# cindytsai/multigrid_poisson_solver

Measured on AMD Instinct MI355X. Metric: vcycle_mlups, higher is better.
Workload: dtype f64; 1 GPU; V(3,3)-cycle N=8192^2 fp64, 11 levels to N=8, red-black GS(1e-7) coarse solve, cycle-file driver (eager, stream smoother: temporally blocked wave-streaming kernels on the large levels, register-tile kernels on the levels 65..1024, one-workgroup LDS kernel below; halos recomputed, neighbours via DPP lane shifts); N=8192, levels=11

## Files before the change

### multigrid_poisson_solver_amd/csrc/mg_stream_impl.h

```cpp
#include <hip/hip_runtime.h>

#include <type_traits>
#include <utility>

#include <algorithm>
#include <cstdlib>
#include <vector>

#include "mg_divconst.h"
#include "mg_internal.h"
#include "mg_lane_ops.h"

#if !defined(MG_REAL) || !defined(MG_REAL_NS)
#error "define MG_REAL (double|float) and MG_REAL_NS (f64|f32) before including mg_stream_impl.h"
#endif

namespace mg {
namespace k {
namespace MG_REAL_NS {

typedef MG_REAL real_t;

constexpr int PF_DEFAULT = 2;
#ifndef MG_WAVES_PER_WG
#define MG_WAVES_PER_WG 4
#endif
constexpr int WAVES_PER_WG = MG_WAVES_PER_WG;
constexpr int MAX_S = 4;
#ifndef MG_PF
#define MG_PF 2
#endif

constexpr bool recompute_instantiated(int pre, int steps)
{
    return MG_PF == 2 && pre >= 1 && steps >= 1 && pre <= MAX_S && steps <= MAX_S && pre + steps <= 6;
}

enum InMode { IN_LOAD = 0, IN_ZERO = 1, IN_PROLONG = 2 };

typedef real_t real2_t __attribute__((ext_vector_type(2)));
typedef real_t real4_t __attribute__((ext_vector_type(4)));

struct StreamParams {
    int N;
    real_t dx2, inv;
    const real_t *in;
    const real_t *F;
    real_t *out;
    real_t *D;
    int d_sign;
    double *part;
    long long *trace;
    int cols4;
    int rows_per_chunk;
    int groups;
    int n_blocks;
    int row_base, rows_local, own_y0, own_y1;
    int norm_y0, norm_y1;
    double *out_wide;
    int coarse_base, coarse_rows;
    int raw_norm;
    int nt_min_n;
    int no_out;
    int pre;
    int fc_base, fc_rows;
    const real_t *coarse;
    int Nc;
    const int *p_orow, *p_ocol;
    const real_t *p_rhi, *p_rlo, *p_chi, *p_clo;
    real_t c_dx, c_dx_rcp;
    real_t *Fc;
    int M;
    const int *r_inv;
    const real_t *r_w;
    const real_t *r_wf;
    const NodeBatchItem *batch;
    int part_stride;
    int n_batch;
    double *const *err_outs;
    real_t cw;
    int wt;
};


typedef const int __attribute__((address_space(4))) *const_int_ptr;
typedef const real_t __attribute__((address_space(4))) *const_real_ptr;
__device__ __forceinline__ int table_i(const int *t, int i) { return ((const_int_ptr)(uintptr_t)t)[i]; }
__device__ __forceinline__ real_t table_d(const real_t *t, int i) { return ((const_real_ptr)(uintptr_t)t)[i]; }

template <int COLS>
struct Row {
    real_t v[COLS];
};

#ifndef MG_ZERO_LEVEL1
#define MG_ZERO_LEVEL1 1
#endif
#ifndef MG_NT_LOADS
#define MG_NT_LOADS 0
#endif
template <int COLS, bool NT = false>
__device__ __forceinline__ Row<COLS> load_row(const real_t *__restrict__ row, unsigned col_bytes)
{
    Row<COLS> r;
    const char *a = reinterpret_cast<const char *>(row) + col_bytes;
    if constexpr (COLS == 2) {
        const real2_t t = NT ? __builtin_nontemporal_load(reinterpret_cast<const real2_t *>(a)) : *reinterpret_cast<const real2_t *>(a);
        r.v[0] = t.x;
        r.v[1] = t.y;
    } else if constexpr (COLS == 4) {
        const real4_t t = NT ? __builtin_nontemporal_load(reinterpret_cast<const real4_t *>(a)) : *reinterpret_cast<const real4_t *>(a);
        r.v[0] = t.x;
        r.v[1] = t.y;
        r.v[2] = t.z;
        r.v[3] = t.w;
    } else {
        r.v[0] = *reinterpret_cast<const real_t *>(a);
    }
    return r;
}

template <int COLS, bool NT>
__device__ __forceinline__ void store_row(real_t *__restrict__ row, unsigned col_bytes, const Row<COLS> &r)
{
    char *a = reinterpret_cast<char *>(row) + col_bytes;
    if constexpr (COLS == 2) {
        real2_t t;
        t.x = r.v[0];
        t.y = r.v[1];
        if constexpr (NT) __builtin_nontemporal_store(t, reinterpret_cast<real2_t *>(a));
        else *reinterpret_cast<real2_t *>(a) = t;
    } else if constexpr (COLS == 4) {
        real4_t t;
        t.x = r.v[0];
        t.y = r.v[1];
        t.z = r.v[2];
        t.w = r.v[3];
        if constexpr (NT) __builtin_nontemporal_store(t, reinterpret_cast<real4_t *>(a));
        else *reinterpret_cast<real4_t *>(a) = t;
    } else {
        *reinterpret_cast<real_t *>(a) = r.v[0];
    }
}

template <int S, bool RESTRICT, int COLS = 2>
struct Halo {
    static constexpr int A = COLS > 2 ? COLS : 2;
    static constexpr int value = (S + (RESTRICT ? 2 : 1) + A - 1) / A * A;
};


template <int NCV>
struct CoarseV {
    real_t v[NCV];
};
template <int NCV>
__device__ __forceinline__ CoarseV<NCV> load_coarse(const real_t *__restrict__ coarse, int Nc, int base, int rows, int row,
                                                    const unsigned (&col)[NCV])
{
    CoarseV<NCV> c;
    int r = row - base;
    r = r < 0 ? 0 : (r < rows - 1 ? r : rows - 1);
    const char *b = reinterpret_cast<const char *>(coarse + (size_t)r * Nc);
#pragma unroll
    for (int q = 0; q < NCV; ++q) c.v[q] = *reinterpret_cast<const real_t *>(b + col[q]);
    return c;
}


template <int NCV>
__device__ __forceinline__ CoarseV<NCV> load_coarse_local(const real_t *__restrict__ coarse, int Nc, int local_row, const unsigned (&col)[NCV])
{
    CoarseV<NCV> c;
    const char *b = reinterpret_cast<const char *>(coarse + (size_t)local_row * Nc);
#pragma unroll
    for (int q = 0; q < NCV; ++q) c.v[q] = *reinterpret_cast<const real_t *>(b + col[q]);
    return c;
}

template <class F, int... K>
__device__ __forceinline__ void unrolled_while(F &&f, std::integer_sequence<int, K...>)
{
    (void)(f(std::integral_constant<int, K>{}) && ...);
}

#ifndef MG_WPE_DOWN
#define MG_WPE_DOWN 0
#endif
template <int S, int COLS, int IN, bool RESTRICT, int PRE>
struct WavesPerSimd {
    static constexpr int min = (MG_WPE_DOWN > 0 && sizeof(real_t) == 8 && COLS == 2 && IN == 1  && RESTRICT && S <= 3) ? MG_WPE_DOWN : 1;
};

#ifndef MG_LDS_RING
#define MG_LDS_RING 1
#endif
#ifndef MG_PACKED_F32
#define MG_PACKED_F32 1
#endif
typedef float pk_t __attribute__((ext_vector_type(2)));
__device__ __forceinline__ pk_t pk(float a, float b)
{
    pk_t r;
    r.x = a;
    r.y = b;
    return r;
}
__device__ __forceinline__ pk_t pk_fma(pk_t a, pk_t b, pk_t c) { return __builtin_elementwise_fma(a, b, c); }
__device__ __forceinline__ pk_t pk_div_by_const(pk_t x, float c, float rc)
{
    const pk_t cc = pk(c, c), rr = pk(rc, rc);
    pk_t q = x * rr;
    pk_t r = pk_fma(-q, cc, x);
    q = pk_fma(r, rr, q);
    r = pk_fma(-q, cc, x);
    return pk_fma(r, rr, q);
}
template <int COLS, int PRE>
struct LdsRing {
    static constexpr bool value = MG_LDS_RING && PRE > 0 && (COLS == 2 || (COLS == 4 && sizeof(real_t) == 4));
};
template <int COLS> struct RingVec { typedef real_t full; typedef real_t half; };
template <> struct RingVec<2> { typedef real2_t full; typedef real_t half; };
template <> struct RingVec<4> { typedef real4_t full; typedef real2_t half; };
template <int COLS>
__device__ __forceinline__ typename RingVec<COLS>::full ring_pack(const Row<COLS> &r)
{
    typename RingVec<COLS>::full t;
    if constexpr (COLS == 1) t = r.v[0];
    else {
#pragma unroll
        for (int j = 0; j < COLS; ++j) t[j] = r.v[j];
    }
    return t;
}
template <int COLS>
__device__ __forceinline__ Row<COLS> ring_unpack(const typename RingVec<COLS>::full &t)
{
    Row<COLS> r;
    if constexpr (COLS == 1) r.v[0] = t;
    else {
#pragma unroll
        for (int j = 0; j < COLS; ++j) r.v[j] = t[j];
    }
    return r;
}
#ifndef MG_PF_UP
#define MG_PF_UP 3
#endif
#ifndef MG_PF_DOWN
#define MG_PF_DOWN 3
#endif
#ifndef MG_WPE_UP
#define MG_WPE_UP 2
#endif

template <int S, int COLS, int IN, bool RESTRICT, int PF = PF_DEFAULT, bool NT = false, int PRE = 0, bool WT = false>
__global__ __launch_bounds__(64 * WAVES_PER_WG) __attribute__((amdgpu_waves_per_eu(LdsRing<COLS, PRE>::value ? MG_WPE_UP : WavesPerSimd<S, COLS, IN, RESTRICT, PRE>::min)))
void k_jacobi_stream(const StreamParams p)
{
    static_assert(COLS == 2 || COLS == 4 || (IN != IN_PROLONG && !RESTRICT), "fused transfer stages need column pairs");
    static_assert(COLS != 4 || sizeof(real_t) == 4, "4 columns per lane = one 16-byte access: fp32 fields only");
    constexpr int NCV = COLS / 2 + 2;
    constexpr int NS = COLS >= 2 ? COLS / 2 : 1;
    static_assert(PRE == 0 || (IN == IN_PROLONG && !RESTRICT), "recomputed pre-smoothing belongs to the fused `1` node");
    static_assert(!WT || (PRE == 0 && sizeof(real_t) == 8), "the weighted sweep: fp64 nodes that store and re-read U");
    constexpr int L = S + PRE;
    constexpr bool LDSR = LdsRing<COLS, PRE>::value;
    constexpr bool HALF = LDSR;
    constexpr bool PACKED = MG_PACKED_F32 && (COLS == 2 || COLS == 4) && sizeof(real_t) == 4;
#ifndef MG_TB_DIRECT
#define MG_TB_DIRECT 0
#endif
    constexpr bool TB_DIRECT = LDSR && MG_TB_DIRECT;
    constexpr int NB = LDSR ? 8 : (PF + L + 2 <= 8 ? 8 : 16);
    constexpr int NFR = LDSR ? (PF < 4 ? 4 : 8) : NB;
    static_assert((LDSR ? L + 2 <= NB : PF + L + 2 <= NB) && PF < 8, "the F ring has NB slots, the U ring 4 or 8");
    static_assert(!LDSR || (IN == IN_PROLONG && !RESTRICT), "the LDS ring belongs to the recomputing `1` node");
    typedef typename RingVec<COLS>::full ring_t;
    typedef typename RingVec<COLS>::half ringh_t;
    __shared__ ring_t s_g[LDSR ? WAVES_PER_WG : 1][LDSR ? NB : 1][LDSR ? 64 : 1];
    __shared__ ringh_t s_f[LDSR ? WAVES_PER_WG : 1][LDSR ? NB : 1][LDSR ? 64 : 1];
    constexpr int W = 64 * COLS;
    constexpr int H = Halo<L, RESTRICT, COLS>::value;
    constexpr int OW = W - 2 * H;

#ifdef MG_STREAM_TRACE
    const long long tr0 = wall_clock64();
#endif
    const int per_xcd = (p.n_blocks + 7) >> 3;
    const int tile = (int)(blockIdx.x & 7) * per_xcd + (int)(blockIdx.x >> 3);
    if (tile >= p.n_blocks) return;
    const real_t *a_in = p.in, *a_F = p.F, *a_coarse = p.coarse;
    real_t *a_out = p.out, *a_Fc = p.Fc;
    double *a_part = p.part;
    if (p.batch) {
        typedef const NodeBatchItem __attribute__((address_space(4))) *item_ptr;
        const item_ptr b = (item_ptr)(uintptr_t)(p.batch + blockIdx.y);
        a_in = static_cast<const real_t *>(b->in);
        a_F = static_cast<const real_t *>(b->F);
        a_coarse = static_cast<const real_t *>(b->coarse);
        a_out = static_cast<real_t *>(b->out);
        a_Fc = static_cast<real_t *>(b->Fc);
        if (a_part) a_part += (size_t)blockIdx.y * (size_t)p.part_stride;
    }
    const int chunk = tile / p.groups;
    const int group = tile - chunk * p.groups;

    const int lane = threadIdx.x & 63;
    const int wave = threadIdx.x >> 6;
    const int strip = group * WAVES_PER_WG + wave;
    const int N = p.N;
    const int own_x0 = strip * OW;
    if (own_x0 >= N) {
        if (a_part && lane == 0) a_part[(size_t)tile * WAVES_PER_WG + wave] = 0.0;
        return;
    }
    const int y0 = p.own_y0 + chunk * p.rows_per_chunk;
    int y1 = y0 + p.rows_per_chunk;
    if (y1 > p.own_y1) y1 = p.own_y1;
    if (y0 >= p.own_y1) return;
    const int av_lo = p.row_base > 0 ? p.row_base : 0;
    const int av_hi = p.row_base + p.rows_local < N ? p.row_base + p.rows_local : N;

    const int xl = own_x0 - H + lane * COLS;
    bool col_in[COLS], col_edge[COLS];
    bool lane_owns = true;
    real_t qc[COLS];
#pragma unroll
    for (int j = 0; j < COLS; ++j) {
        const int x = xl + j;
        col_in[j] = x >= 0 && x < N;
        col_edge[j] = x <= 0 || x >= N - 1;
        lane_owns = lane_owns && x >= own_x0 && x < own_x0 + OW && x < N;
        qc[j] = col_edge[j] ? real_t(0.0) : (WT ? p.cw : real_t(0.25));
    }
    int nm_even[COLS], nm_odd[COLS];
#pragma unroll
    for (int j = 0; j < COLS; ++j) {
        const bool mine = lane_owns && !col_edge[j];
        nm_even[j] = (mine && ((xl + j) & 1) == 0) ? -1 : 0;
        nm_odd[j] = (mine && ((xl + j) & 1) != 0) ? -1 : 0;
    }
    const bool lane_loads = col_in[0] && col_in[COLS - 1];
    const real_t dx2 = p.dx2, inv = p.inv;
    const bool want_res = RESTRICT || p.D != nullptr || p.part != nullptr;
    const unsigned col_off = (unsigned)(xl < 0 ? 0 : (xl > N - COLS ? N - COLS : xl)) * (unsigned)sizeof(real_t);
    const unsigned col_st = (unsigned)(xl < 0 ? 0 : xl) * (unsigned)sizeof(real_t);
    const unsigned row_bytes = (unsigned)N * (unsigned)sizeof(real_t);

    unsigned pc_col[NCV];
    int pc_cell[COLS];
    real_t pc_hi[COLS], pc_lo[COLS];
    real_t hA[COLS], hB[COLS];
#pragma unroll
    for (int q = 0; q < NCV; ++q) pc_col[q] = 0u;
#pragma unroll
    for (int j = 0; j < COLS; ++j) {
        pc_cell[j] = 0;
        pc_hi[j] = pc_lo[j] = hA[j] = hB[j] = real_t(0.0);
    }
    int c_row = -0x40000000;
    if constexpr (IN == IN_PROLONG) {
        if (lane_loads) {
            const int pc_base = p.p_ocol[xl];
            const int last = p.Nc - 1;
#pragma unroll
            for (int j = 0; j < COLS; ++j) {
                pc_cell[j] = p.p_ocol[xl + j] - pc_base;
                pc_hi[j] = p.p_chi[xl + j];
                pc_lo[j] = p.p_clo[xl + j];
            }
#pragma unroll
            for (int q = 0; q < NCV; ++q) pc_col[q] = (unsigned)(pc_base + q < last ? pc_base + q : last) * (unsigned)sizeof(real_t);
        }
    }
    auto interpolate = [&](const CoarseV<NCV> &c, real_t (&h)[COLS]) {
#pragma unroll
        for (int j = 0; j < COLS; ++j) {
            real_t ca = c.v[0], cb = c.v[1];
#pragma unroll
            for (int q = 1; q + 1 < NCV; ++q) {
                const bool here = pc_cell[j] == q;
                ca = here ? c.v[q] : ca;
                cb = here ? c.v[q + 1] : cb;
            }
            h[j] = ca * pc_hi[j] + cb * pc_lo[j];
        }
    };

    int rc_col[NS];
    bool rc_shift[NS];
    real_t rw_a[NS], rw_b[NS];
    Row<COLS> d_prev;
#pragma unroll
    for (int j = 0; j < COLS; ++j) d_prev.v[j] = 0.0;
#pragma unroll
    for (int q = 0; q < NS; ++q) {
        rc_col[q] = -1;
        rc_shift[q] = false;
        rw_a[q] = rw_b[q] = real_t(0.0);
    }
    if constexpr (RESTRICT) {
        if (lane_owns) {
#pragma unroll
            for (int q = 0; q < NS; ++q) {
                const int ca = p.r_inv[xl + 2 * q], cb = p.r_inv[xl + 2 * q + 1];
                rc_col[q] = ca >= 0 ? ca : cb;
                rc_shift[q] = ca < 0 && cb >= 0;
                if (rc_col[q] >= 0) {
                    rw_a[q] = p.r_w[rc_col[q]];
                    rw_b[q] = real_t(1.0) - rw_a[q];
                }
            }
        }
    }
    const bool first_col_lane = RESTRICT && lane_owns && xl == 0;
    const bool last_col_lane = RESTRICT && lane_owns && xl + COLS == N;
    if constexpr (RESTRICT) {
        for (int edge = 0; edge < 2; ++edge) {
            if (edge == 0 ? (y0 != 0) : (y1 != N)) continue;
            real_t *row = a_Fc + (size_t)((edge == 0 ? 0 : p.M - 1) - p.fc_base) * p.M;
#pragma unroll
            for (int q = 0; q < NS; ++q)
                if (rc_col[q] >= 0) row[rc_col[q]] = 0.0;
            if (first_col_lane) row[0] = 0.0;
            if (last_col_lane) row[p.M - 1] = 0.0;
        }
    }
    real_t ms[COLS];
#pragma unroll
    for (int j = 0; j < COLS; ++j) ms[j] = col_edge[j] ? real_t(0.0) : (p.d_sign < 0 ? real_t(-1.0) : real_t(1.0));

    constexpr bool EVEN_START = COLS >= 2;
    const int y0e = EVEN_START ? (y0 & ~1) : y0;
    const int y_first = y0e - (L + 1);
    const int T = (y1 - y0e) + 2 * (L + 1) + (RESTRICT ? 1 : 0);
    const int y_end = y_first + T;

    int tb_own = -1, tbn_own = -1;
    real_t tb_yh = 0.0, tb_yl = 0.0, tbn_yh = 0.0, tbn_yl = 0.0;
    int tb_rc = -1, tbn_rc = -1;
    real_t tb_rw = 0.0, tbn_rw = 0.0;
    auto load_own_block = [&](int first_row) {
        const int y = first_row + lane;
        const bool ok = y >= av_lo && y < av_hi && y < y_end;
        const int yc = y < 0 ? 0 : (y < N ? y : N - 1);
        const int v = p.p_orow[yc];
        tbn_own = ok ? v : -1;
    };
    auto load_weight_block = [&](int first_row) {
        const int y = first_row + lane;
        const int yc = y < 0 ? 0 : (y < N ? y : N - 1);
        tbn_yh = p.p_rhi[yc];
        tbn_yl = p.p_rlo[yc];
    };
    auto load_restrict_block = [&](int first_row) {
        const int y = first_row + lane;
        const bool ok = y >= y0 && y < y1;
        const int yc = y < 0 ? 0 : (y < N ? y : N - 1);
        const int v = p.r_inv[yc];
        const real_t w = p.r_wf[yc];
        tbn_rc = ok ? v : -1;
        tbn_rw = w;
    };
    const int yp_first = y_first - PRE;
    if constexpr (IN == IN_PROLONG) {
        load_own_block(yp_first);
        tb_own = tbn_own;
        load_weight_block(yp_first);
        tb_yh = tbn_yh;
        tb_yl = tbn_yl;
    }
    if constexpr (RESTRICT) {
        load_restrict_block(y_first - (L + 2));
        tb_rc = tbn_rc;
        tb_rw = tbn_rw;
    }

    Row<COLS> older[L + 1], newer[L + 1];
#pragma unroll
    for (int l = 0; l <= L; ++l)
#pragma unroll
        for (int j = 0; j < COLS; ++j) older[l].v[j] = newer[l].v[j] = 0.0;
    constexpr int NU = PF < 4 ? 4 : 8;
    Row<COLS> fr[NFR], pu[NU];
    CoarseV<NCV> pc[NU];
    int q_own[NU];
#pragma unroll
    for (int k = 0; k < NFR; ++k)
#pragma unroll
        for (int j = 0; j < COLS; ++j) fr[k].v[j] = 0.0;
#pragma unroll
    for (int k = 0; k < NU; ++k) {
#pragma unroll
        for (int j = 0; j < COLS; ++j) pu[k].v[j] = 0.0;
#pragma unroll
        for (int q = 0; q < NCV; ++q) pc[k].v[q] = 0.0;
        q_own[k] = -1;
    }

    if constexpr (LDSR) {
#pragma unroll
        for (int k = 0; k < NB; ++k) {
            s_g[wave][k][lane] = ring_t(real_t(0.0));
            s_f[wave][k][lane] = ringh_t(real_t(0.0));
        }
    }

    const char *in_b = reinterpret_cast<const char *>(a_in), *f_b = reinterpret_cast<const char *>(a_F);
    const int yc_first = y_first < av_lo ? av_lo : (y_first < av_hi ? y_first : av_hi - 1);
    unsigned long long ld_off = (unsigned long long)(yc_first - p.row_base) * row_bytes;
    int ld_t = 0;
    long long st_off = (long long)(y_first - L - p.row_base) * (long long)row_bytes;
    const unsigned inner_rows = (unsigned)(av_hi - av_lo - 1);

    auto fetch = [&](int u8) {
        if constexpr (IN != IN_ZERO && PRE == 0) pu[u8 % NU] = load_row<COLS, (MG_NT_LOADS >= 2)>(reinterpret_cast<const real_t *>(in_b + ld_off), col_off);
        fr[u8 % NFR] = load_row<COLS, (MG_NT_LOADS >= 1)>(reinterpret_cast<const real_t *>(f_b + ld_off), col_off);
        if constexpr (IN == IN_PROLONG) {
            const int own_s = lane_value(tb_own, ld_t & 63);
            q_own[u8 % NU] = own_s;
            const int cr = own_s + 1 - p.coarse_base;
            const int crc = cr < 0 ? 0 : (cr < p.coarse_rows - 1 ? cr : p.coarse_rows - 1);
            pc[u8 % NU] = load_coarse_local<NCV>(a_coarse, p.Nc, crc, pc_col);
        }
        ++ld_t;
        ld_off += ((unsigned)(y_first + ld_t - av_lo - 1) < inner_rows) ? row_bytes : 0u;
    };
#pragma unroll
    for (int k = 0; k < PF; ++k) fetch(k);

    if constexpr (IN == IN_PROLONG) {
        const int ys = yp_first > av_lo ? yp_first : av_lo;
        if (ys < av_hi && ys < y_end) {
            const int i0 = table_i(p.p_orow, ys);
            const CoarseV<NCV> c0 = load_coarse<NCV>(a_coarse, p.Nc, p.coarse_base, p.coarse_rows, i0, pc_col);
            interpolate(c0, hB);
            c_row = i0 - 1;
        }
    }

#ifdef MG_STREAM_TRACE
    const long long tr1 = wall_clock64();
#endif
    Row<COLS> gq[L + 1];
#pragma unroll
    for (int l = 0; l <= L; ++l)
#pragma unroll
        for (int j = 0; j < COLS; ++j) gq[l].v[j] = 0.0;
    double acc = 0.0;
    const unsigned rows_own = (unsigned)(y1 - y0), rows_norm = (unsigned)(p.norm_y1 - p.norm_y0);
    int nm_k0[COLS], nm_k1[COLS];
    const bool first_odd = ((y_first - L - 1) & 1) != 0;
    {
#pragma unroll
        for (int j = 0; j < COLS; ++j) {
            nm_k0[j] = first_odd ? nm_odd[j] : nm_even[j];
            nm_k1[j] = first_odd ? nm_even[j] : nm_odd[j];
        }
    }

    for (int t0 = 0; t0 < T; t0 += NB) {
        if ((t0 & 63) == 64 - NB) {
            if constexpr (IN == IN_PROLONG && !TB_DIRECT) {
                load_own_block(yp_first + t0 + NB);
                load_weight_block(yp_first + t0 + NB);
            }
            if constexpr (RESTRICT) load_restrict_block(y_first + t0 + NB - (L + 2));
        }
        if ((t0 & 63) == 0 && t0 > 0) {
            if constexpr (IN == IN_PROLONG && TB_DIRECT) {
                load_weight_block(yp_first + t0);
            }
            if constexpr (IN == IN_PROLONG) {
                tb_yh = tbn_yh;
                tb_yl = tbn_yl;
            }
            if constexpr (RESTRICT) {
                tb_rc = tbn_rc;
                tb_rw = tbn_rw;
            }
        }
        auto row_step = [&](auto k_tag) -> bool {
            constexpr int k = decltype(k_tag)::value;
            const int t = t0 + k;
            if (!LDSR && k > 0 && t >= T) return false;
            const int yin = y_first + t;
            Row<COLS> nw;
            if constexpr (IN == IN_ZERO || PRE > 0) {
#pragma unroll
                for (int j = 0; j < COLS; ++j) nw.v[j] = 0.0;
            } else {
                nw = pu[k % NU];
            }
            const int own_i = q_own[k % NU];
            if constexpr (IN == IN_PROLONG) {
                if (k == NB - PF && (t0 & 63) == 64 - NB) {
                    if constexpr (TB_DIRECT) load_own_block(yp_first + t0 + NB);
                    tb_own = tbn_own;
                }
                if (own_i >= 0 && own_i != c_row) {
                    asm volatile("" ::);
#pragma unroll
                    for (int j = 0; j < COLS; ++j) hA[j] = hB[j];
                    c_row = own_i;
                    interpolate(pc[k % NU], hB);
                }
            }
            fetch((k + PF) % NB);

            auto add_prolongation = [&](Row<COLS> &row) {
                if (own_i >= 0) {
                    const real_t own_yh = lane_value(tb_yh, t & 63), own_yl = lane_value(tb_yl, t & 63);
                    const real_t c_dx = p.c_dx, c_rcp = p.c_dx_rcp;
                    if constexpr (PACKED) {
#pragma unroll
                        for (int j = 0; j < COLS; j += 2) {
                            const pk_t yh2 = pk((float)own_yh, (float)own_yh), yl2 = pk((float)own_yl, (float)own_yl);
                            const pk_t num = pk((float)hA[j], (float)hA[j + 1]) * yh2 + pk((float)hB[j], (float)hB[j + 1]) * yl2;
                            const pk_t pv = pk_div_by_const(pk_div_by_const(num, (float)c_dx, (float)c_rcp), (float)c_dx, (float)c_rcp);
                            const pk_t sum = pk((float)row.v[j], (float)row.v[j + 1]) + pv;
                            row.v[j] = sum.x;
                            row.v[j + 1] = sum.y;
                        }
                    } else {
#pragma unroll
                        for (int j = 0; j < COLS; ++j) {
                            const real_t num = hA[j] * own_yh + hB[j] * own_yl;
                            const real_t pv = div_by_const(div_by_const(num, c_dx, c_rcp), c_dx, c_rcp);
                            row.v[j] = row.v[j] + pv;
                        }
                    }
                }
            };
            if constexpr (IN == IN_PROLONG && PRE == 0) add_prolongation(nw);

#pragma unroll
            for (int l = 1; l <= L; ++l) {
                const int y = yin - l;
                const int inner = ((unsigned)(y - 1) < (unsigned)(N - 2)) ? -1 : 0;
                const Row<COLS> c = newer[l - 1], so = older[l - 1];
                Row<COLS> g;
                if constexpr (LDSR) {
                    g = gq[l];
                } else {
                    const Row<COLS> &f = fr[(k - l + NB) % NB];
#pragma unroll
                    for (int j = 0; j < COLS; ++j) g.v[j] = dx2 * f.v[j];
                }
                const real_t west0 = from_lane_below(c.v[COLS - 1]);
                const real_t east_last = from_lane_above(c.v[0]);
                Row<COLS> o;
                if constexpr (PACKED) {
#pragma unroll
                    for (int P = 0; P < COLS / 2; ++P) {
                        const int a = 2 * P, b = 2 * P + 1;
                        const pk_t q2 = pk((float)hi_bits_and(qc[a], inner), (float)hi_bits_and(qc[b], inner));
                        const pk_t g2 = pk((float)g.v[a], (float)g.v[b]);
                        pk_t o2;
                        if ((IN == IN_ZERO || PRE > 0) && MG_ZERO_LEVEL1 && l == 1) {
                            o2 = pk_fma(q2, -g2, pk(0.0f, 0.0f));
                        } else {
                            const pk_t c2 = pk((float)c.v[a], (float)c.v[b]);
                            const pk_t e2 = pk((float)c.v[b], (float)(b == COLS - 1 ? east_last : c.v[b < COLS - 1 ? b + 1 : 0]));
                            const pk_t w2 = pk((float)(a == 0 ? west0 : c.v[a > 0 ? a - 1 : 0]), (float)c.v[a]);
                            pk_t t2 = pk((float)nw.v[a], (float)nw.v[b]) + pk((float)so.v[a], (float)so.v[b]);
                            t2 = t2 + e2;
                            t2 = t2 + w2;
                            t2 = pk_fma(pk(-4.0f, -4.0f), c2, t2) - g2;
                            o2 = pk_fma(q2, t2, c2);
                        }
                        o.v[a] = o2.x;
                        o.v[b] = o2.y;
                    }
                    older[l - 1] = c;
                    newer[l - 1] = nw;
                    nw = o;
                    if constexpr (IN == IN_PROLONG && PRE > 0) {
                        if (l == PRE) add_prolongation(nw);
                    }
                    continue;
                }
                if constexpr ((IN == IN_ZERO || PRE > 0) && MG_ZERO_LEVEL1) {
                    if (l == 1) {
#pragma unroll
                        for (int j = 0; j < COLS; ++j) {
                            if constexpr (WT) o.v[j] = fused_mul_add(inner ? qc[j] : real_t(0.0), -g.v[j], real_t(0.0));
                            else o.v[j] = fused_mul_add(hi_bits_and(qc[j], inner), -g.v[j], real_t(0.0));
                        }
                        older[l - 1] = c;
                        newer[l - 1] = nw;
                        nw = o;
                        if constexpr (IN == IN_PROLONG && PRE > 0) {
                            if (l == PRE) add_prolongation(nw);
                        }
                        continue;
                    }
                }
#pragma unroll
                for (int j = 0; j < COLS; ++j) {
                    const real_t w = j == 0 ? west0 : c.v[j > 0 ? j - 1 : 0];
                    const real_t e = j == COLS - 1 ? east_last : c.v[j < COLS - 1 ? j + 1 : 0];
                    const real_t t4 = minus4(nw.v[j] + so.v[j] + e + w, c.v[j]) - g.v[j];
                    if constexpr (WT) o.v[j] = c.v[j] + (inner ? qc[j] : real_t(0.0)) * t4;
                    else o.v[j] = fused_mul_add(hi_bits_and(qc[j], inner), t4, c.v[j]);
                }
                older[l - 1] = c;
                newer[l - 1] = nw;
                nw = o;
                if constexpr (IN == IN_PROLONG && PRE > 0) {
                    if (l == PRE) add_prolongation(nw);
                }
            }

            if constexpr (LDSR) {
                const Row<COLS> &fin = fr[k % NFR];
                Row<COLS> gin;
#pragma unroll
                for (int j = 0; j < COLS; ++j) gin.v[j] = dx2 * fin.v[j];
                s_g[wave][k % NB][lane] = ring_pack<COLS>(gin);
                constexpr int par = (k + L + 1) & 1;
                if constexpr (COLS == 2) {
                    s_f[wave][k % NB][lane] = fin.v[par];
                } else {
                    ringh_t h;
                    h.x = fin.v[par];
                    h.y = fin.v[par + 2];
                    s_f[wave][k % NB][lane] = h;
                }
#pragma unroll
                for (int l = 1; l <= L; ++l) {
                    gq[l] = ring_unpack<COLS>(s_g[wave][(k + 1 - l + 2 * NB) % NB][lane]);
                }
            }

            {
                const int y = yin - L;
                if ((unsigned)(y - y0) < rows_own && lane_owns && !p.no_out) {
                    if (sizeof(real_t) != sizeof(double) && p.out_wide) {
                        double *w = reinterpret_cast<double *>(reinterpret_cast<char *>(p.out_wide) + 2 * st_off + 2u * col_st);
                        typedef double wide2_t __attribute__((ext_vector_type(2)));
                        if constexpr (COLS % 2 == 0) {
#pragma unroll
                            for (int j = 0; j < COLS; j += 2) {
                                wide2_t t;
                                t.x = (double)nw.v[j];
                                t.y = (double)nw.v[j + 1];
                                if (COLS == 2) __builtin_nontemporal_store(t, reinterpret_cast<wide2_t *>(w + j));
                                else *reinterpret_cast<wide2_t *>(w + j) = t;
                            }
                        } else {
#pragma unroll
                            for (int j = 0; j < COLS; ++j) __builtin_nontemporal_store((double)nw.v[j], w + j);
                        }
                    } else {
                        store_row<COLS, NT>(reinterpret_cast<real_t *>(reinterpret_cast<char *>(a_out) + st_off), col_st, nw);
                    }
                }
            }

            if (want_res) {
                const int y = yin - L - 1;
                const bool mine_row = (unsigned)(y - y0) < rows_own;
                const int inner = ((unsigned)(y - 1) < (unsigned)(N - 2)) ? -1 : 0;
                const int cm = (mine_row && (unsigned)(y - p.norm_y0) < rows_norm) ? inner : 0;
                const Row<COLS> c = newer[L], so = older[L];
                if constexpr (HALF) {
                    const ringh_t fh = s_f[wave][(k - L - 1 + 2 * NB) % NB][lane];
#pragma unroll
                    for (int j = k & 1; j < COLS; j += 2) {
                        real_t fv;
                        if constexpr (COLS == 2) fv = fh;
                        else fv = fh[j >> 1];
                        const real_t w = j == 0 ? from_lane_below(c.v[COLS - 1]) : c.v[j > 0 ? j - 1 : 0];
                        const real_t e = j == COLS - 1 ? from_lane_above(c.v[0]) : c.v[j < COLS - 1 ? j + 1 : 0];
                        const real_t r = inv * minus4(nw.v[j] + so.v[j] + e + w, c.v[j]) - fv;
                        const int am = ((lane_owns && !col_edge[j]) ? -1 : 0) & cm;
                        acc += fabs(bits_and((double)r, am));
                    }
                    older[L] = newer[L];
                    newer[L] = nw;
                    st_off += row_bytes;
                    return true;
                }
                const Row<COLS> &f = fr[(k - L - 1 + 2 * NB) % NFR];
                const real_t west0 = from_lane_below(c.v[COLS - 1]);
                const real_t east_last = from_lane_above(c.v[0]);
                Row<COLS> d;
#pragma unroll
                for (int j = 0; j < COLS; ++j) {
                    const real_t w = j == 0 ? west0 : c.v[j > 0 ? j - 1 : 0];
                    const real_t e = j == COLS - 1 ? east_last : c.v[j < COLS - 1 ? j + 1 : 0];
                    const real_t r = inv * minus4(nw.v[j] + so.v[j] + e + w, c.v[j]) - f.v[j];
                    if constexpr (RESTRICT) {
                        d.v[j] = r * hi_bits_and(ms[j], inner);
                    } else {
                        d.v[j] = r;
                    }
                    if constexpr (EVEN_START) {
                        if ((j & 1) == (k & 1)) acc += fabs(bits_and((double)r, ((lane_owns && !col_edge[j]) ? -1 : 0) & cm));
                    } else {
                        const int am = ((k & 1) ? nm_k1[j] : nm_k0[j]) & cm;
                        acc += fabs(bits_and((double)r, am));
                    }
                }
                if constexpr (!RESTRICT) {
                    if (mine_row && lane_owns && p.D) {
                        Row<COLS> ds;
#pragma unroll
                        for (int j = 0; j < COLS; ++j) {
                            const real_t dv = (inner != 0 && !col_edge[j]) ? d.v[j] : real_t(0.0);
                            ds.v[j] = p.d_sign < 0 ? -dv : dv;
                        }
                        store_row<COLS, false>(reinterpret_cast<real_t *>(reinterpret_cast<char *>(p.D) + (st_off - (long long)row_bytes)), col_st, ds);
                    }
                } else {
                    if (mine_row && lane_owns && p.D)
                        store_row<COLS, false>(reinterpret_cast<real_t *>(reinterpret_cast<char *>(p.D) + (st_off - (long long)row_bytes)), col_st, d);
                }

                if constexpr (RESTRICT) {
                    const int rc_row = lane_value(tb_rc, t & 63);
                    if (rc_row >= 0) {
                        const real_t wc = lane_value(tb_rw, t & 63), wd = real_t(1.0) - wc;
                        const real_t p_up = from_lane_above(d_prev.v[0]);
                        const real_t q_up = from_lane_above(d.v[0]);
                        real_t *crow = a_Fc + (size_t)(rc_row - p.fc_base) * p.M;
#pragma unroll
                        for (int q = 0; q < NS; ++q) {
                            const real_t p_next = q + 1 < NS ? d_prev.v[q + 1 < NS ? 2 * q + 2 : 0] : p_up;
                            const real_t q_next = q + 1 < NS ? d.v[q + 1 < NS ? 2 * q + 2 : 0] : q_up;
                            const real_t u0 = rc_shift[q] ? d_prev.v[2 * q + 1] : d_prev.v[2 * q];
                            const real_t u1 = rc_shift[q] ? p_next : d_prev.v[2 * q + 1];
                            const real_t u2 = rc_shift[q] ? d.v[2 * q + 1] : d.v[2 * q];
                            const real_t u3 = rc_shift[q] ? q_next : d.v[2 * q + 1];
                            const real_t vc = rw_b[q] * wd * u0 + rw_a[q] * wd * u1 + wc * rw_b[q] * u2 + rw_a[q] * wc * u3;
                            if (rc_col[q] >= 0) crow[rc_col[q]] = vc;
                        }
                        if (first_col_lane) crow[0] = 0.0;
                        if (last_col_lane) crow[p.M - 1] = 0.0;
                    }
                    d_prev = d;
                }
            }
            older[L] = newer[L];
            newer[L] = nw;
            st_off += row_bytes;
            return true;
        };
        unrolled_while(row_step, std::make_integer_sequence<int, NB>{});
    }
#ifdef MG_STREAM_TRACE
    if (p.trace && (threadIdx.x & 63) == 0) {
        const long long tr2 = wall_clock64();
        long long *rec = p.trace + 8 + 4 * ((size_t)tile * WAVES_PER_WG + wave);
        rec[0] = tr0;
        rec[1] = tr1;
        rec[2] = tr2;
        rec[3] = (long long)blockIdx.x;
        if (tile == p.n_blocks / 2 && wave == 0) {
            p.trace[0] = tr0;
            p.trace[1] = tr1;
            p.trace[2] = tr2;
            p.trace[3] = T;
        }
    }
#endif
    if (a_part) {
#pragma unroll
        for (int o = 32; o > 0; o >>= 1) acc += __shfl_down(acc, o, 64);
        if (lane == 0) a_part[(size_t)tile * WAVES_PER_WG + wave] = acc;
    }
}

#ifndef MG_STREAM_KERNEL_ONLY
template <int S, int COLS, int IN, bool RESTRICT, int PF = PF_DEFAULT, bool NT = false, int PRE = 0, bool WT = false>
void launch_k(hipStream_t s, StreamParams p, double *err_out)
{
    static int blocks_per_cu = 0;
    if (blocks_per_cu == 0) {
        int n = 0;
        if (hipOccupancyMaxActiveBlocksPerMultiprocessor(&n, k_jacobi_stream<S, COLS, IN, RESTRICT, PF, NT, PRE, WT>, 64 * WAVES_PER_WG, 0) != hipSuccess || n < 1) {
            (void)hipGetLastError();
            n = 2;
        }
        blocks_per_cu = n > 8 ? 8 : n;
    }
    const int N = p.N;
    const int own = p.own_y1 - p.own_y0;
    if (own <= 0) return;
    constexpr int OW = 64 * COLS - 2 * Halo<S + PRE, RESTRICT, COLS>::value;
    const int strips = (N + OW - 1) / OW;
    const int groups = (strips + WAVES_PER_WG - 1) / WAVES_PER_WG;
    static const int resident_pct = [] { const char *e = getenv("MG_RESIDENT_PCT"); return e ? atoi(e) : 100; }();
    const int resident = ctx().n_cu * blocks_per_cu * resident_pct / 100;
    const int nb = p.batch ? p.n_batch : 1;
    int chunks = resident / (groups * nb);
    static const int min_rows_forced = [] { const char *e = getenv("MG_MIN_ROWS"); return e ? atoi(e) : 0; }();
    const int min_rows = min_rows_forced ? min_rows_forced : (N <= 256 ? 2 : N <= 1024 ? 4 : 8);
    const int max_chunks = (own + min_rows - 1) / min_rows;
    if (chunks > max_chunks) chunks = max_chunks;
    if (chunks < 1) chunks = 1;
    int rows = (own + chunks - 1) / chunks;
    static const int rows_cap = [] { const char *e = getenv("MG_MAX_ROWS"); return e ? atoi(e) : 0; }();
    if (rows_cap > 0 && rows > rows_cap) rows = rows_cap;
    if (LdsRing<COLS, PRE>::value) {
        const int march = rows + 2 * (S + PRE + 1);
        rows += (8 - march % 8) % 8;
    } else if (COLS >= 2) {
        rows += rows & 1;
    }
    chunks = (own + rows - 1) / rows;
    p.rows_per_chunk = rows;
    p.groups = groups;
    p.n_blocks = chunks * groups;
    p.part = nullptr;
#ifdef MG_STREAM_TRACE
    static long long *trace_dev = nullptr;
    if (!trace_dev) (void)hipMalloc((void **)&trace_dev, (8 + 4 * 4 * 4096) * sizeof(long long));
    (void)hipMemsetAsync(trace_dev, 0, (8 + 4 * 4 * 4096) * sizeof(long long), s);
    p.trace = trace_dev;
#endif
    const size_t n_part = (size_t)p.n_blocks * WAVES_PER_WG;
    const bool want_norm = err_out || (p.batch && p.err_outs);
    if (want_norm) {
        p.part = norm_partials(n_part * (size_t)nb);
        if (!p.part) return;
    }
    p.part_stride = (int)n_part;
    const int grid = ((p.n_blocks + 7) / 8) * 8;
    hipLaunchKernelGGL((k_jacobi_stream<S, COLS, IN, RESTRICT, PF, NT, PRE, WT>), dim3(grid, nb), dim3(64 * WAVES_PER_WG), 0, s, p);
#ifdef MG_STREAM_TRACE
    {
        long long t[4];
        (void)hipStreamSynchronize(s);
        (void)hipMemcpy(t, trace_dev, sizeof t, hipMemcpyDeviceToHost);
        fprintf(stderr, "[stream trace] N=%d IN=%d R=%d tiles=%d rows/chunk=%d: prologue %.2f us, %lld steps %.2f us (%.3f us/step)\n", N, IN, (int)RESTRICT,
                p.n_blocks, rows, (t[1] - t[0]) * 0.01, t[3], (t[2] - t[1]) * 0.01, (t[2] - t[1]) * 0.01 / (double)t[3]);
        if (N >= 4096 && p.n_blocks <= 4096) {
            const size_t nw = (size_t)p.n_blocks * WAVES_PER_WG;
            std::vector<long long> all(4 * nw);
            (void)hipMemcpy(all.data(), trace_dev + 8, all.size() * sizeof(long long), hipMemcpyDeviceToHost);
            long long t_min = 0x7fffffffffffffffll, t_max = 0;
            std::vector<double> start, life, endt;
            for (size_t w = 0; w < nw; ++w) {
                if (all[4 * w] == 0) continue;
                if (all[4 * w] < t_min) t_min = all[4 * w];
                if (all[4 * w + 2] > t_max) t_max = all[4 * w + 2];
            }
            double xcd_end[8] = {0}, xcd_start[8] = {0};
            for (size_t w = 0; w < nw; ++w) {
                if (all[4 * w] == 0) continue;
                start.push_back((all[4 * w] - t_min) * 0.01);
                endt.push_back((all[4 * w + 2] - t_min) * 0.01);
                life.push_back((all[4 * w + 2] - all[4 * w]) * 0.01);
                const int x = (int)(all[4 * w + 3] & 7);
                if (endt.back() > xcd_end[x]) xcd_end[x] = endt.back();
                if (start.back() > xcd_start[x]) xcd_start[x] = start.back();
            }
            auto pct = [](std::vector<double> v, double q) { std::sort(v.begin(), v.end()); return v[(size_t)(q * (v.size() - 1))]; };
            fprintf(stderr, "   waves %zu: start p50 %.1f p99 %.1f max %.1f us | lifetime p1 %.1f p50 %.1f p99 %.1f max %.1f | end p1 %.1f p50 %.1f p99 %.1f max %.1f | span %.1f us\n",
                    nw, pct(start, .5), pct(start, .99), pct(start, 1.0), pct(life, .01), pct(life, .5), pct(life, .99), pct(life, 1.0), pct(endt, .01),
                    pct(endt, .5), pct(endt, .99), pct(endt, 1.0), (t_max - t_min) * 0.01);
            fprintf(stderr, "   last wave per XCD ends at:");
            for (int x = 0; x < 8; ++x) fprintf(stderr, " %.1f", xcd_end[x]);
            fprintf(stderr, " us\n");
        }
    }
#endif
    if (p.batch && p.err_outs) {
        for (int i = 0; i < nb; ++i)
            if (p.err_outs[i]) norm_finish(s, p.part + (size_t)i * n_part, n_part, p.raw_norm ? -1 : N, p.err_outs[i]);
    } else if (err_out) {
        norm_finish(s, p.part, n_part, p.raw_norm ? -1 : N, err_out);
    }
}

template <int S, int PF>
void launch_variant(hipStream_t s, const StreamParams &p, double *err_out)
{
    const bool restrict_out = p.Fc != nullptr, prolong_in = p.coarse != nullptr, zero = p.in == nullptr;
    const bool nt = p.N >= p.nt_min_n;
    if constexpr (sizeof(real_t) == 4) {
        if (p.cols4 && !(prolong_in && p.pre)) {
            if (restrict_out) {
                if (zero) launch_k<S, 4, IN_ZERO, true, PF>(s, p, err_out);
                else launch_k<S, 4, IN_LOAD, true, PF>(s, p, err_out);
            } else if (prolong_in) {
                if (nt) launch_k<S, 4, IN_PROLONG, false, PF, true>(s, p, err_out);
                else launch_k<S, 4, IN_PROLONG, false, PF>(s, p, err_out);
            } else {
                if (zero) launch_k<S, 4, IN_ZERO, false, PF>(s, p, err_out);
                else launch_k<S, 4, IN_LOAD, false, PF>(s, p, err_out);
            }
            return;
        }
    }
    if constexpr (sizeof(real_t) == 8) {
        if (p.wt) {
            if (p.N % 2 != 0) {
                if (zero) launch_k<S, 1, IN_ZERO, false, PF, false, 0, true>(s, p, err_out);
                else launch_k<S, 1, IN_LOAD, false, PF, false, 0, true>(s, p, err_out);
            } else if (restrict_out) {
                if (zero) launch_k<S, 2, IN_ZERO, true, (PF == 2 && S <= 3 ? MG_PF_DOWN : PF), false, 0, true>(s, p, err_out);
                else launch_k<S, 2, IN_LOAD, true, PF, false, 0, true>(s, p, err_out);
            } else if (prolong_in) {
                if (p.pre != 0) fail(MG_ERR_UNSUPPORTED, "jacobi_stream: no recomputing `1` node for the weighted sweep");
                else if (nt) launch_k<S, 2, IN_PROLONG, false, PF, true, 0, true>(s, p, err_out);
                else launch_k<S, 2, IN_PROLONG, false, PF, false, 0, true>(s, p, err_out);
            } else {
                if (zero) launch_k<S, 2, IN_ZERO, false, PF, false, 0, true>(s, p, err_out);
                else launch_k<S, 2, IN_LOAD, false, PF, false, 0, true>(s, p, err_out);
            }
            return;
        }
    }
    if (p.N % 2 != 0) {
        if (zero) launch_k<S, 1, IN_ZERO, false, PF>(s, p, err_out);
        else launch_k<S, 1, IN_LOAD, false, PF>(s, p, err_out);
    } else if (restrict_out) {
        if (zero) launch_k<S, 2, IN_ZERO, true, (PF == 2 && S <= 3 ? MG_PF_DOWN : PF)>(s, p, err_out);
        else launch_k<S, 2, IN_LOAD, true, PF>(s, p, err_out);
    } else if (prolong_in) {
        if (p.pre != 0) {
            bool done = false;
            auto with_pre = [&](auto pre_tag) {
                constexpr int PRE = decltype(pre_tag)::value;
                if constexpr (recompute_instantiated(PRE, S) && PF == 2) {
                    if (p.pre == PRE && !done) {
                        constexpr int PFU = LdsRing<2, PRE>::value ? MG_PF_UP : PF;
                        if (nt) launch_k<S, 2, IN_PROLONG, false, PFU, true, PRE>(s, p, err_out);
                        else launch_k<S, 2, IN_PROLONG, false, PFU, false, PRE>(s, p, err_out);
                        done = true;
                    }
                }
            };
            with_pre(std::integral_constant<int, 1>{});
            with_pre(std::integral_constant<int, 2>{});
            with_pre(std::integral_constant<int, 3>{});
            with_pre(std::integral_constant<int, 4>{});
            if (!done) fail(MG_ERR_UNSUPPORTED, "jacobi_stream: no recomputing `1` node for %d + %d sweeps, prefetch depth %d", p.pre, S, PF);
            return;
        }
        if (nt) launch_k<S, 2, IN_PROLONG, false, PF, true>(s, p, err_out);
        else launch_k<S, 2, IN_PROLONG, false, PF>(s, p, err_out);
    } else {
        if (zero) launch_k<S, 2, IN_ZERO, false, PF>(s, p, err_out);
        else launch_k<S, 2, IN_LOAD, false, PF>(s, p, err_out);
    }
}

template <int S>
void launch_steps(hipStream_t s, const StreamParams &p, double *err_out)
{
    if constexpr (S <= 3 && MG_PF == 3) launch_variant<S, 3>(s, p, err_out);
    else launch_variant<S, 2>(s, p, err_out);
}


inline void run(hipStream_t s, const SmoothNode<real_t> &nd)
{
    const int N = nd.N, steps = nd.steps, pre = nd.pre;
    const RowWindow *fine_w = nd.fine_w;
    if (nd.batch && (fine_w || nd.coarse_w || nd.fc_w || nd.D || nd.out_wide || nd.batch->n < 1)) {
        fail(MG_ERR_ARG, "jacobi_stream: a batch of instances runs whole grids without a stored residual");
        return;
    }
    if (pre != 0 && !(recompute_instantiated(pre, steps) && nd.coarse && !nd.Fc)) {
        fail(MG_ERR_ARG, "jacobi_stream: recomputed pre-smoothing exists for pre + steps <= 6 sweeps of the fused `1` node (pre=%d steps=%d)", pre, steps);
        return;
    }
    if (nd.cw != 0.25 && (pre != 0 || sizeof(real_t) != 8)) {
        fail(MG_ERR_ARG, "jacobi_stream: the weighted sweep runs fp64 nodes that store and re-read U");
        return;
    }
    if (pre != 0 && nd.D) {
        fail(MG_ERR_ARG, "jacobi_stream: the recomputing `1` node forms the error norm only, it stores no residual");
        return;
    }
    if (steps < 1 || steps > MAX_S) {
        fail(MG_ERR_ARG, "jacobi_stream: %d sweeps per launch (1..%d)", steps, MAX_S);
        return;
    }
    if ((nd.coarse || nd.Fc) && (N < 4 || N % 2 != 0)) {
        fail(MG_ERR_ARG, "jacobi_stream: fused transfer stages need an even grid size (N=%d)", N);
        return;
    }
    StreamParams p = {};
    if (nd.batch) {
        p.batch = nd.batch->dev;
        p.n_batch = nd.batch->n;
        p.err_outs = nd.batch->err_outs;
    }
    p.N = N;
    p.dx2 = nd.dx2;
    p.inv = nd.inv;
    p.in = nd.in;
    p.F = nd.F;
    p.out = nd.out;
    p.out_wide = nd.out_wide;
    p.pre = pre;
    p.no_out = nd.no_out ? 1 : 0;
    p.cw = (real_t)nd.cw;
    p.wt = nd.cw != 0.25 ? 1 : 0;
    p.D = nd.D;
    p.d_sign = nd.d_sign;
    p.row_base = fine_w ? fine_w->base : 0;
    p.rows_local = fine_w ? fine_w->rows : N;
    p.own_y0 = fine_w ? fine_w->own_lo : 0;
    p.own_y1 = fine_w ? fine_w->own_hi : N;
    p.norm_y0 = fine_w && fine_w->norm_lo >= 0 ? fine_w->norm_lo : p.own_y0;
    p.norm_y1 = fine_w && fine_w->norm_lo >= 0 ? fine_w->norm_hi : p.own_y1;
    p.raw_norm = fine_w ? 1 : 0;
    static const int cols4_min = [] { const char *e = getenv("MG_F32_COLS4_MIN_N"); return e ? atoi(e) : 8192; }();
    p.cols4 = (sizeof(real_t) == 4 && N % 4 == 0 && N >= cols4_min && (!nd.coarse || nd.pt->fusable4)) ? 1 : 0;
    static const int nt_min = [] { const char *e = getenv("MG_NT_MIN_N"); return e ? atoi(e) : 8192; }();
    p.nt_min_n = nt_min;
    if (nd.coarse) {
        const ProlongTable &pt = *nd.pt;
        p.coarse_base = nd.coarse_w ? nd.coarse_w->base : 0;
        p.coarse_rows = nd.coarse_w ? nd.coarse_w->rows : nd.Nc;
        p.coarse = nd.coarse;
        p.Nc = nd.Nc;
        p.p_orow = pt.owner_row;
        p.p_ocol = pt.owner_col;
        p.p_rhi = weights_as(real_t(), pt.row_hi, pt.row_hi_f);
        p.p_rlo = weights_as(real_t(), pt.row_lo, pt.row_lo_f);
        p.p_chi = weights_as(real_t(), pt.col_hi, pt.col_hi_f);
        p.p_clo = weights_as(real_t(), pt.col_lo, pt.col_lo_f);
        p.c_dx = (real_t)pt.c_dx;
        p.c_dx_rcp = (real_t)1 / p.c_dx;
    }
    if (nd.Fc) {
        const RestrictTable &rt = *nd.rt;
        p.fc_base = nd.fc_w ? nd.fc_w->base : 0;
        p.fc_rows = nd.fc_w ? nd.fc_w->rows : nd.M;
        p.Fc = nd.Fc;
        p.M = nd.M;
        p.r_inv = rt.inv;
        p.r_w = weights_as(real_t(), rt.w, rt.w_f);
        p.r_wf = weights_as(real_t(), rt.inv_w, rt.inv_w_f);
    }
    switch (steps) {
        case 1: launch_steps<1>(s, p, nd.err); break;
        case 2: launch_steps<2>(s, p, nd.err); break;
        case 3: launch_steps<3>(s, p, nd.err); break;
        default: launch_steps<4>(s, p, nd.err); break;
    }
}

#endif

}
}
}
```

Before: 787,300 MLUPS.

## Pack stream waves densely across strips and chunks, widen edge strip ownership

Waves are now mapped as a flat global index over strips times chunks instead of per-workgroup strip groups, so no workgroup carries idle waves when the strip count is not a multiple of the waves per workgroup. The strip count is recomputed so the first and last strips own their halo columns at the domain boundary, which can reduce the number of strips needed. The chunk count is chosen against the packed block count to fill resident slots. Waves in a workgroup may now come from different row chunks, and a debug geometry print is added.

```diff
diff --git a/multigrid_poisson_solver_amd/csrc/mg_stream_impl.h b/multigrid_poisson_solver_amd/csrc/mg_stream_impl.h
--- a/multigrid_poisson_solver_amd/csrc/mg_stream_impl.h
+++ b/multigrid_poisson_solver_amd/csrc/mg_stream_impl.h
@@ -53,7 +53,8 @@
     long long *trace;
     int cols4;
     int rows_per_chunk;
-    int groups;
+    int strips;
+    int n_waves;
     int n_blocks;
     int row_base, rows_local, own_y0, own_y1;
     int norm_y0, norm_y1;
@@ -304,18 +305,19 @@
         a_Fc = static_cast<real_t *>(b->Fc);
         if (a_part) a_part += (size_t)blockIdx.y * (size_t)p.part_stride;
     }
-    const int chunk = tile / p.groups;
-    const int group = tile - chunk * p.groups;
-
     const int lane = threadIdx.x & 63;
-    const int wave = threadIdx.x >> 6;
-    const int strip = group * WAVES_PER_WG + wave;
+    const int wave = __builtin_amdgcn_readfirstlane((int)(threadIdx.x >> 6));
+    const int gw = tile * WAVES_PER_WG + wave;
+    if (gw >= p.n_waves) {
+        if (a_part && lane == 0) a_part[gw] = 0.0;
+        return;
+    }
+    const int chunk = gw / p.strips;
+    const int strip = gw - chunk * p.strips;
     const int N = p.N;
-    const int own_x0 = strip * OW;
-    if (own_x0 >= N) {
-        if (a_part && lane == 0) a_part[(size_t)tile * WAVES_PER_WG + wave] = 0.0;
-        return;
-    }
+    const int win_x0 = strip * OW;
+    const int own_x0 = strip == 0 ? 0 : win_x0 + H;
+    const int own_x1 = strip == p.strips - 1 ? N : win_x0 + W - H;
     const int y0 = p.own_y0 + chunk * p.rows_per_chunk;
     int y1 = y0 + p.rows_per_chunk;
     if (y1 > p.own_y1) y1 = p.own_y1;
@@ -323,7 +325,7 @@
     const int av_lo = p.row_base > 0 ? p.row_base : 0;
     const int av_hi = p.row_base + p.rows_local < N ? p.row_base + p.rows_local : N;
 
-    const int xl = own_x0 - H + lane * COLS;
+    const int xl = win_x0 + lane * COLS;
     bool col_in[COLS], col_edge[COLS];
     bool lane_owns = true;
     real_t qc[COLS];
@@ -332,7 +334,7 @@
         const int x = xl + j;
         col_in[j] = x >= 0 && x < N;
         col_edge[j] = x <= 0 || x >= N - 1;
-        lane_owns = lane_owns && x >= own_x0 && x < own_x0 + OW && x < N;
+        lane_owns = lane_owns && x >= own_x0 && x < own_x1;
         qc[j] = col_edge[j] ? real_t(0.0) : (WT ? p.cw : real_t(0.25));
     }
     int nm_even[COLS], nm_odd[COLS];
@@ -854,7 +856,7 @@
 #ifdef MG_STREAM_TRACE
     if (p.trace && (threadIdx.x & 63) == 0) {
         const long long tr2 = wall_clock64();
-        long long *rec = p.trace + 8 + 4 * ((size_t)tile * WAVES_PER_WG + wave);
+        long long *rec = p.trace + 8 + 4 * (size_t)gw;
         rec[0] = tr0;
         rec[1] = tr1;
         rec[2] = tr2;
@@ -870,7 +872,7 @@
     if (a_part) {
 #pragma unroll
         for (int o = 32; o > 0; o >>= 1) acc += __shfl_down(acc, o, 64);
-        if (lane == 0) a_part[(size_t)tile * WAVES_PER_WG + wave] = acc;
+        if (lane == 0) a_part[gw] = acc;
     }
 }
 
@@ -890,13 +892,15 @@
     const int N = p.N;
     const int own = p.own_y1 - p.own_y0;
     if (own <= 0) return;
-    constexpr int OW = 64 * COLS - 2 * Halo<S + PRE, RESTRICT, COLS>::value;
-    const int strips = (N + OW - 1) / OW;
-    const int groups = (strips + WAVES_PER_WG - 1) / WAVES_PER_WG;
+    constexpr int W = 64 * COLS;
+    constexpr int OW = W - 2 * Halo<S + PRE, RESTRICT, COLS>::value;
+    const int strips = N <= W ? 1 : 1 + (N - W + OW - 1) / OW;
     static const int resident_pct = [] { const char *e = getenv("MG_RESIDENT_PCT"); return e ? atoi(e) : 100; }();
     const int resident = ctx().n_cu * blocks_per_cu * resident_pct / 100;
     const int nb = p.batch ? p.n_batch : 1;
-    int chunks = resident / (groups * nb);
+    auto blocks_of = [&](int c) { return (strips * c + WAVES_PER_WG - 1) / WAVES_PER_WG; };
+    int chunks = resident * WAVES_PER_WG / (strips * nb);
+    while (chunks > 1 && blocks_of(chunks) * nb > resident) --chunks;
     static const int min_rows_forced = [] { const char *e = getenv("MG_MIN_ROWS"); return e ? atoi(e) : 0; }();
     const int min_rows = min_rows_forced ? min_rows_forced : (N <= 256 ? 2 : N <= 1024 ? 4 : 8);
     const int max_chunks = (own + min_rows - 1) / min_rows;
@@ -913,8 +917,9 @@
     }
     chunks = (own + rows - 1) / rows;
     p.rows_per_chunk = rows;
-    p.groups = groups;
-    p.n_blocks = chunks * groups;
+    p.strips = strips;
+    p.n_waves = strips * chunks;
+    p.n_blocks = blocks_of(chunks);
     p.part = nullptr;
 #ifdef MG_STREAM_TRACE
     static long long *trace_dev = nullptr;
@@ -929,6 +934,17 @@
         if (!p.part) return;
     }
     p.part_stride = (int)n_part;
+    static const bool show_geometry = getenv("MG_STREAM_GEOMETRY") != nullptr;
+    if (show_geometry) {
+        static std::vector<long long> seen;
+        const long long key = ((long long)N << 32) ^ ((long long)nb << 20) ^ ((long long)p.own_y0 << 10) ^ (long long)own;
+        if (std::find(seen.begin(), seen.end(), key) == seen.end()) {
+            seen.push_back(key);
+            fprintf(stderr, "[stream geometry] N=%d S=%d PRE=%d IN=%d R=%d COLS=%d: %d strips x %d chunks x %d inst = %d waves in %d blocks (resident %d), %d rows/chunk, march %d steps\n",
+                    N, S, PRE, IN, (int)RESTRICT, COLS, strips, chunks, nb, strips * chunks * nb, p.n_blocks * nb, resident, rows,
+                    rows + 2 * (S + PRE + 1) + (RESTRICT ? 1 : 0));
+        }
+    }
     const int grid = ((p.n_blocks + 7) / 8) * 8;
     hipLaunchKernelGGL((k_jacobi_stream<S, COLS, IN, RESTRICT, PF, NT, PRE, WT>), dim3(grid, nb), dim3(64 * WAVES_PER_WG), 0, s, p);
 #ifdef MG_STREAM_TRACE
```

Result: no change. 795,200 MLUPS, median of 6 (+1.0%).
